# neobotix/neo_mpc_planner2

Measured on AMD Instinct MI355X. Metric: MPC solves/sec (control_steps=3, 500x500 costmap), higher is better.
Workload: dtype f64

## Files before the change

### neo_mpc_planner2_amd/csrc/neo_mpc_kernels.hip

```cpp
#include <hip/hip_runtime.h>
#include <hip/hip_ext.h>
#include <math.h>
#include <stdint.h>
#include <stdlib.h>

#include "neo_mpc_device.h"
#include "wave_ops.h"
#include "fast_math.h"
#include "solver_context.h"
#include "solver_rules.h"
#include "costmap.h"
#include "feasible_set.h"
#include "rollout.h"
#include "riccati.h"
#include "adjoint.h"
#include "tangent_cone.h"
#include "dense_newton.h"
#include "lbfgs.h"
#include "cell_scan.h"

namespace neo_mpc {
namespace {

constexpr int kStallIterations = NEO_RULE_STALL_ITERATIONS;
constexpr int kBlockedRun = NEO_RULE_BLOCKED_RUN;
constexpr double kBlockedStep = NEO_RULE_BLOCKED_STEP;
constexpr double kFinalFracGaussNewton = NEO_RULE_FINAL_FRAC_GN;
constexpr double kWindowStep = NEO_RULE_WINDOW_STEP;
constexpr int kClosingRun = NEO_RULE_CLOSING_RUN;
constexpr int kLateIteration = NEO_RULE_LATE_ITERATION;

#ifdef NEO_MPC_PHASE_TIMING
#ifdef NEO_MPC_SEGMENT_TIMING
#define NEO_SEGMENT_DECL unsigned long long seg_t0 = 0, seg_t1 = 0, seg_scan = 0, seg_scan_at = 0
#define NEO_SEGMENT(k) seg_t##k = wall_clock64()
#define NEO_SEGMENT_SCAN_BEGIN() seg_scan_at = wall_clock64(); seg_scan = seg_scan_at
#define NEO_SEGMENT_SCAN_END() seg_scan = wall_clock64() - seg_scan
#define NEO_SEGMENT_DUMP()                                                                                   \
  {                                                                                                          \
    SolveArgs ad;                                                                                            \
    fresh_args<kSteps, kStaticTile, kLayoutSteps, kRouted>(ad);                                              \
    const int nvd = 3 * ad.p.n;                                                                              \
    if (ad.solution && lane_again() == 0 && nvd >= 9) {                                                      \
      ad.solution[(size_t)b * nvd + 4] = (double)seg_t0; ad.solution[(size_t)b * nvd + 5] = (double)seg_t1;  \
      ad.solution[(size_t)b * nvd + 3] = (double)seg_scan; ad.solution[(size_t)b * nvd + 2] = (double)seg_scan_at; \
    }                                                                                                        \
  }
#else
#define NEO_SEGMENT_DECL
#define NEO_SEGMENT(k)
#define NEO_SEGMENT_SCAN_BEGIN()
#define NEO_SEGMENT_SCAN_END()
#define NEO_SEGMENT_DUMP()
#endif
#define NEO_WAVE_START const unsigned long long wave_t0 = wall_clock64()
#define NEO_WAVE_END_ARGS(args)                                                                     \
  if ((args).solution && lane == 0 && (args).p.n >= 3) {                                            \
    const int nvw = 3 * (args).p.n;                                                                \
    unsigned int hw_id, xcc_id;                                                                    \
    asm volatile("s_getreg_b32 %0, hwreg(HW_REG_HW_ID)" : "=s"(hw_id));                            \
    asm volatile("s_getreg_b32 %0, hwreg(HW_REG_XCC_ID)" : "=s"(xcc_id));                          \
    (args).solution[(size_t)b * nvw + 6] = (double)wave_t0;                                        \
    (args).solution[(size_t)b * nvw + 7] = (double)wall_clock64();                                 \
    (args).solution[(size_t)b * nvw + 8] = (double)hw_id + 4294967296.0 * (double)(xcc_id & 15u);  \
  }
#define NEO_PHASE_DECL long long phase_clock[8]
#define NEO_PHASE(k) phase_clock[k] = clock64()
#define NEO_PHASE_DUMP()                                                                            \
  if (it == 2 && a.solution && lane == 0)                                                          \
    for (int k = 0; k < 6; ++k) a.solution[(size_t)b * nv + k] = (double)(phase_clock[k + 1] - phase_clock[k])
#else
#define NEO_WAVE_START
#define NEO_WAVE_END_ARGS(args)
#define NEO_SEGMENT_DECL
#define NEO_SEGMENT(k)
#define NEO_SEGMENT_SCAN_BEGIN()
#define NEO_SEGMENT_SCAN_END()
#define NEO_SEGMENT_DUMP()
#define NEO_PHASE_DECL
#define NEO_PHASE(k)
#define NEO_PHASE_DUMP()
#endif
constexpr int kNewtonMaxSteps = 8;

constexpr int kRoutedSteps = 3;
constexpr LdsLayout make_routed_stagewise_layout() {
  LdsLayout l = make_lds_layout(kRoutedSteps, 0, true, true);
  constexpr LdsLayout dense = make_lds_layout(kRoutedSteps, 4, false);
  l.tile = dense.tile;
  l.total_bytes = dense.total_bytes;
  return l;
}
static_assert(make_lds_layout(kRoutedSteps, 0, true, true).tile <= make_lds_layout(kRoutedSteps, 4, false).tile,
              "the stage-wise arrays of three stages fit in front of the dense kernel's reach tile");
static_assert(make_lds_layout(kRoutedSteps, 0, true, true).gr == make_lds_layout(kRoutedSteps, 4, false).gr,
              "records, iterate and gradients share their offsets");
template <int kSteps, int kStaticTile, int kLayoutSteps, bool kRouted = false>
__device__ __forceinline__ void fresh_args(SolveArgs& a) {
  auto kp = (const __attribute__((address_space(4))) char*)__builtin_amdgcn_kernarg_segment_ptr();
  asm volatile("" : "+s"(kp));
  a = *(const SolveArgs*)kp;
  if (kRouted) {
    constexpr LdsLayout kLayout = make_routed_stagewise_layout();
    const int tile_w = a.lds.tile_w, tile_h = a.lds.tile_h, reach = a.lds.reach;
    a.lds = kLayout;
    a.lds.tile_w = tile_w; a.lds.tile_h = tile_h; a.lds.reach = reach;
    a.p.n = kRoutedSteps;
  } else if (kSteps || kStaticTile) {
    constexpr LdsLayout kStaticLayout = make_lds_layout(kLayoutSteps, kSteps ? 4 : 0, false);
    const int tile_w = a.lds.tile_w, tile_h = a.lds.tile_h, reach = a.lds.reach;
    a.lds = kStaticLayout;
    a.lds.tile_w = tile_w; a.lds.tile_h = tile_h; a.lds.reach = reach;
    if (kSteps) a.p.n = kSteps;
  }
}
__device__ __forceinline__ void own_loop_params(SolveArgs& a) {
  auto own = [](double& v) { asm volatile("" : "+s"(v)); };
  own(a.p.dt); own(a.p.wt_n); own(a.p.wo_n); own(a.p.wc_n); own(a.p.wterm_o); own(a.p.r);
  own(a.p.lo[2]); own(a.p.hi[2]);
  own(a.map.origin_x); own(a.map.origin_y); own(a.map.resolution); own(a.map.inv_resolution);
}
template <bool kVectorPose>
__device__ __forceinline__ void ctx_from_lds(const SolveArgs& a, const double* L, Ctx& c) {
  const double* P = L + a.lds.prob;
  const double* t = L + a.lds.tol;
  c.cx = lane_value(P[P_CARROT_X], 0); c.cy = lane_value(P[P_CARROT_Y], 0);
  c.tyaw = lane_value(t[T_TYAW], 0); c.fyaw = lane_value(t[T_FYAW], 0);
  c.v0 = lane_value(P[P_VEL], 0); c.v1 = lane_value(P[P_VEL + 1], 0); c.v2 = lane_value(P[P_VEL + 2], 0);
  c.c0 = t[T_C0]; c.s0 = t[T_S0]; c.X0 = P[P_CUR_X]; c.Y0 = P[P_CUR_Y];
  if (kVectorPose) asm volatile("" : "+v"(c.c0), "+v"(c.s0), "+v"(c.X0), "+v"(c.Y0));
  else { c.c0 = lane_value(c.c0, 0); c.s0 = lane_value(c.s0, 0); c.X0 = lane_value(c.X0, 0); c.Y0 = lane_value(c.Y0, 0); }
  const int* ti = reinterpret_cast<const int*>(t + T_TILE);
  c.tile_x0 = uniform_int(ti[0]); c.tile_y0 = uniform_int(ti[1]); c.tile_geom = uniform_int(ti[2]);
  c.konst = 0.0; c.true_yaw = 0.0;
}

struct SolveCarry {
  int flags;
  bool cold;
  bool wall_in_reach;
  double f = INFINITY;
  int it = 0, nfev = 1, status = NEO_MPC_STATUS_MAX_ITER;
};

template <int kSteps, bool kTame, int kStaticTile, int kLayoutSteps>
__device__ __forceinline__ bool solve_setup(double* L, uint32_t b, int lane, SolveCarry& s) {
  constexpr bool kCovered = kStaticTile > 0;
  int flags;
  bool cold = true;
  {
    SolveArgs a;
    fresh_args<kSteps, kStaticTile, kLayoutSteps>(a);
    const DevParams& p = a.p;
    const int n = kSteps ? kSteps : p.n, nv = 3 * n;
    load_records(a, L, b, lane);
    if (uniform_int(reinterpret_cast<const int*>(L + a.lds.prob)[PI_SKIP]) == 1) { skip_instance(a, b, lane); return false; }
    select_map(a.map, L + a.lds.prob);
    flags = reset_and_warm(a, L, b, lane) ? NEO_MPC_FLAG_RESET : 0;
    const double fcost = footprint_cost(a, L, b, lane);
    if (lane == 0) L[a.lds.prob + P_FOOTPRINT] = fcost;
    Ctx c;
    make_ctx_wave(p, a.map, L + a.lds.prob, fcost, c, lane);
    load_tile(a, c, L, lane);
    s.wall_in_reach = (c.tile_geom & kTileWall) != 0;
    if (s.wall_in_reach) flags |= NEO_MPC_FLAG_WALL_IN_REACH;
    if (lane == 0) {
      double* t = L + a.lds.tol;
      t[T_XTOL] = p.xtol; t[T_EARLY] = p.early_tol; t[T_FINAL] = p.final_tol; t[T_FTOL] = p.ftol;
      t[T_STALL] = p.stall_step; t[T_WTOL] = p.wtol; t[T_WTOL_LATE] = p.wtol_late; t[T_KINK] = p.kink_radius;
      t[T_KONST] = c.konst; t[T_TRUE_YAW] = c.true_yaw;
      t[T_HOP_DROP] = p.hop_min_drop; t[T_HOP_RANGE] = p.hop_range;
      t[T_BTOL_MAP] = p.btol_map; t[T_BTOL_FREE] = p.btol_free;
      reinterpret_cast<int*>(t + T_HOP_STAGE)[kHopLanes] = 0;
      t[T_C0] = c.c0; t[T_S0] = c.s0; t[T_TYAW] = c.tyaw; t[T_FYAW] = c.fyaw;
      int* ti = reinterpret_cast<int*>(t + T_TILE);
      ti[0] = c.tile_x0; ti[1] = c.tile_y0; ti[2] = c.tile_geom;
    }
    double* u = L + a.lds.u;
    for (int i = lane; i < n; i += kLanes) project_block<kTame>(p, u[3 * i], u[3 * i + 1], u[3 * i + 2]);
    WAVE_SYNC();
    for (int k = 0; k < nv; ++k) cold = cold && (u[k] == 0.0);
    ctx_from_lds<false>(a, L, c);
    {
      double* S = L + a.lds.state;
      int* Si = reinterpret_cast<int*>(S);
      const bool has_prev = uniform_int(Si[SI_HAS_PREV]) == 1 && !(flags & NEO_MPC_FLAG_RESET);
      WAVE_SYNC();
      if (lane == 0) {
        double q0 = has_prev ? S[S_PREV_U0] : u[nv - 3], q1 = has_prev ? S[S_PREV_U0 + 1] : u[nv - 2], q2 = has_prev ? S[S_PREV_U0 + 2] : u[nv - 1];
        project_block<kTame>(p, q0, q1, q2);
        S[S_PREV_U0] = q0; S[S_PREV_U0 + 1] = q1; S[S_PREV_U0 + 2] = q2;
        Si[SI_HAS_PREV] = 0;
      }
      WAVE_SYNC();
    }
    if (!cold && n > 1 && !(p.compat & kCompatNoUnshift) && p.max_it < kDumpGradient) {
      const double* A0 = L + a.lds.state + S_PREV_U0;
      double ts = 0.0;
      const double fs = rollout_cost<kSteps, kTame, kCovered>(
          a, c, L,
          [&](int i, double& b0, double& b1, double& b2) {
            const double* src = lane == 1 ? (i == 0 ? A0 : u + 3 * (i - 1)) : u + 3 * i;
            b0 = src[0]; b1 = src[1]; b2 = src[2];
          },
          NoRecord(), &ts);
      const double f_warm = lane_value(fs, 0), f_alt = lane_value(fs, 1);
      const bool free_both = lane_value(ts, 0) == 0.0 && lane_value(ts, 1) == 0.0;
      if (f_alt < f_warm && free_both) {
        double v0 = 0.0, v1 = 0.0, v2 = 0.0;
        const int k0 = lane, k1 = lane + kLanes, k2 = lane + 2 * kLanes;
        if (k0 < nv) v0 = k0 >= 3 ? u[k0 - 3] : A0[k0];
        if (k1 < nv) v1 = u[k1 - 3];
        if (k2 < nv) v2 = u[k2 - 3];
        WAVE_SYNC();
        if (k0 < nv) u[k0] = v0;
        if (k1 < nv) u[k1] = v1;
        if (k2 < nv) u[k2] = v2;
      } else if (f_alt < f_warm && lane == 0) {
        reinterpret_cast<int*>(L + a.lds.state)[SI_HAS_PREV] = kAltArmed;
      }
      WAVE_SYNC();
    }
  }
  s.flags = flags; s.cold = cold;
  return true;
}

template <int kMinWavesPerSimd, int kSteps, int kDir, bool kTame, int kStaticTile, int kLayoutSteps, bool kRouted = false>
__device__ __forceinline__ bool solve_search(double* L, uint32_t b, SolveCarry& sc) {
  constexpr bool kCovered = kStaticTile > 0;
  constexpr bool kNewton = kDir == 1;
  constexpr bool kRiccati = kDir == 2;
  constexpr bool kSecond = kDir != 0;
  constexpr bool kBlockedRule = kNewton || kRouted;
  static_assert(!kRiccati || kSteps == 0 || kRouted, "the stage-wise direction: run-time-sized, or the routed kernel's control_steps-3 branch");
  static_assert(!kRouted || (kRiccati && kSteps == kRoutedSteps), "the routed branch is the stage-wise one, three stages in registers");
  constexpr int kFew = (kRiccati && kSteps > 0) ? kSteps : 0;
  constexpr int kNwSteps = !kNewton ? 1 : kSteps ? kSteps : kNewtonMaxSteps;
  constexpr bool kVectorPose = kTame;
  constexpr int kRegSteps = kSteps ? kSteps : 1;
  constexpr int kPairs = kSteps ? 4 : NEO_MPC_MAX_LBFGS_MEMORY;
  double f = sc.f;
  const bool cold = sc.cold;
  int npairs = 0, head = 0, nfev = sc.nfev, it = sc.it, status = sc.status, stall = 0;
  int blocked_run = 0;
  int nblocked = 1;
  double u_term = 0.0;
  double gain1 = INFINITY, gain2 = INFINITY;
  bool final_step = false;
  double alpha = 1.0;
  bool scanned = false;
  int nscans = 0;
  bool scan_only = false;
  auto lane_again = []() {
    int zero;
    asm volatile("v_mov_b32 %0, 0" : "=v"(zero));
    return (int)__builtin_amdgcn_mbcnt_hi(~0u, __builtin_amdgcn_mbcnt_lo(~0u, (unsigned)zero));
  };
  NEO_SEGMENT_DECL;
  NEO_SEGMENT(0);
  for (;;) {
  SolveArgs a;
  fresh_args<kSteps, kStaticTile, kLayoutSteps, kRouted>(a);
  own_loop_params(a);
  select_map(a.map, L + a.lds.prob);
  const DevParams& p = a.p;
  const int n = kSteps ? kSteps : p.n, nv = 3 * n, mem = p.mem;
  double cand[3 * kRegSteps], cand_sn[kRegSteps], cand_cs[kRegSteps];
  bool have_trig = false;
  Ctx c;
  ctx_from_lds<kVectorPose>(a, L, c);
  double* u = L + a.lds.u;
  double* gs = L + a.lds.gs;
  double* gt = L + a.lds.gt;
  double* gr = L + a.lds.gr;
  double* d = L + a.lds.d;
  double* u_prev = L + a.lds.u_prev;
  double* gt_prev = L + a.lds.gt_prev;
  double* u_new = L + a.lds.u_new;
  double* ACS = L + a.lds.cs;
  double* ASN = L + a.lds.sn;
  int* AMODE = reinterpret_cast<int*>(L + a.lds.mode);
  static_assert(2 * 7 >= kNewtonRecord, "Newton records do not fit the step arrays");

  if (!scanned && nscans == 0) {
    const int lane = lane_again();
    for (int i = lane; i < n; i += kLanes) { AMODE[4 * i + 2] = 0; AMODE[4 * i + 3] = 0; }
    if (kRouted && lane == 0) L[a.lds.tol + T_KINK] = p.kink_radius_stagewise;
    alpha = kRiccati ? fmax(1.0, n * 0.125) : 1.0;
    if (kFew && lane == 0) { double* t = L + a.lds.tol; t[T_GAIN1] = INFINITY; t[T_GAIN2] = INFINITY; t[T_ALPHA] = alpha; }
    if (kRiccati && lane == 0) L[a.lds.tol + T_MU] = n > 8 ? (double)(n - 8) * 0.125 : 0.0;
  }
  bool v_feasible = false;
  if (kRiccati) {
    double b0 = c.v0, b1 = c.v1, b2 = c.v2;
    asm volatile("" : "+v"(b0), "+v"(b1), "+v"(b2));
    project_block<kTame>(p, b0, b1, b2);
    v_feasible = b0 == c.v0 && b1 == c.v1 && b2 == c.v2;
  }
  double my_scale;
  {
    int l0 = lane_again();
    my_scale = kRiccati ? 0.0 : lane_scale<kSecond>(l0);
  }
  for (; it < p.max_it && !scan_only; ++it) {
    int lane = lane_again();
    const bool exact_step = kRiccati && nblocked == 0;
    int tol_off = a.lds.tol;
    asm volatile("" : "+s"(tol_off));
    const double* TOL = L + tol_off;
    NEO_PHASE_DECL;
    NEO_PHASE(0);
    constexpr int kVars = 3 * kNwSteps;
    const int nvr = kSteps ? kVars : nv;
    bool free_path = false;
    int nhops = 0;
    float hc[kVars];
    float newton_sol = 0.0f;
    if (kNewton) {
      double hcol[kSteps ? kVars : 1];
      const double hstep = 1e-6, inv_h = 1.0 / hstep;
      double pcs[kNwSteps], psn[kNwSteps];
      double x = 0.0, y = 0.0, th = 0.0;
    #pragma unroll
      for (int i = 0; i < kNwSteps; ++i) {
        if (kSteps || i < n) {
          const double vx = u[3 * i] + (lane == 3 * i ? hstep : 0.0);
          const double vy = u[3 * i + 1] + (lane == 3 * i + 1 ? hstep : 0.0);
          const double w = u[3 * i + 2] + (lane == 3 * i + 2 ? hstep : 0.0);
          th += w * p.dt;
          sincos_heading<kTame>(th, &psn[i], &pcs[i]);
          x += (vx * pcs[i] - vy * psn[i]) * p.dt;
          y += (vx * psn[i] + vy * pcs[i]) * p.dt;
        }
      }
      double SX = 0.0, SY = 0.0, ST = 0.0;
    #pragma unroll
      for (int k = kNwSteps - 1; k >= 0; --k) {
        if (kSteps || k < n) {
          const double vx = u[3 * k] + (lane == 3 * k ? hstep : 0.0);
          const double vy = u[3 * k + 1] + (lane == 3 * k + 1 ? hstep : 0.0);
          const double w = u[3 * k + 2] + (lane == 3 * k + 2 ? hstep : 0.0);
          const double pdx = (vx * pcs[k] - vy * psn[k]) * p.dt, pdy = (vx * psn[k] + vy * pcs[k]) * p.dt;
          double prt = -2.0 * p.wo_n * (c.tyaw - th);
          if (k == n - 1) prt += -2.0 * p.wterm_o * (c.fyaw - th);
          SX += -2.0 * p.wt_n * (c.cx - x); SY += -2.0 * p.wt_n * (c.cy - y);
          ST += prt - pdy * SX + pdx * SY;
          const double g0 = p.dt * (pcs[k] * SX + psn[k] * SY), g1 = p.dt * (-psn[k] * SX + pcs[k] * SY),
                       g2 = p.dt * ST;
          if (kSteps) {
            hcol[3 * k] = g0; hcol[3 * k + 1] = g1; hcol[3 * k + 2] = g2;
          } else {
            const double b0 = lane_value(g0, 63), b1 = lane_value(g1, 63), b2 = lane_value(g2, 63);
            if (lane == 63) { gs[3 * k] = b0; gs[3 * k + 1] = b1; gs[3 * k + 2] = b2; }
            hc[3 * k] = (float)((g0 - b0) * inv_h);
            hc[3 * k + 1] = (float)((g1 - b1) * inv_h);
            hc[3 * k + 2] = (float)((g2 - b2) * inv_h);
          }
          x -= pdx; y -= pdy; th -= w * p.dt;
        } else {
          hc[3 * k] = 0.0f; hc[3 * k + 1] = 0.0f; hc[3 * k + 2] = 0.0f;
        }
      }
      if (kSteps) {
    #pragma unroll
        for (int j = 0; j < kVars; ++j) {
          const double base = lane_value(hcol[j], 63);
          if (lane == 63) gs[j] = base;
          hc[j] = (float)((hcol[j] - base) * inv_h);
        }
      }
      WAVE_SYNC();
    }
    else if (!kSteps || kRiccati) adjoint_by_scans<kTame, kRiccati, kFew>(a, c, L, exact_step, lane, n, free_path, nhops);
    else adjoint_short_sweep<kSteps, kTame>(a, c, L, have_trig, lane, n);
    NEO_PHASE(1);
    const bool my_corner = tangent_cone_pass<kTame, kNewton, kRiccati>(a, c, L, TOL[T_KINK], lane, n);
    WAVE_SYNC();
    const bool corner_any = kSecond && !kTame && __ballot(my_corner) != 0ull && (kRiccati ? free_path : (it > 0 && u_term == 0.0));
    NEO_PHASE(2);
    if (p.max_it == kDumpGradient) {
      for (int k = lane; k < nv; k += kLanes) a.solution[(size_t)b * nv + k] = gt[k];
      return true;
    }
    if (kSecond && it == 0 && cold) {
      if (kRiccati) { for (int k = lane; k < nv; k += kLanes) d[k] = -gr[k]; }
      else if (lane < nvr) d[lane] = -gr[lane];
      if (kRiccati) for (int i = lane; i < n; i += kLanes) AMODE[4 * i + 3] = 0;
      WAVE_SYNC();
    } else if (kRiccati) {
      riccati_prepare(a, c, L, n, lane, v_feasible, (float)TOL[T_MU]);
      WAVE_SYNC();
      if (corner_any) riccati_keep_linear_terms(a, L, n, lane, true);
      auto sweep = [&]() {
        riccati_sweep<float, (kMinWavesPerSimd < 4), kFew>(a, L, n, lane);
        riccati_finish(a, c, L, n, lane);
      };
      sweep();
      if (!kTame && corner_any && repin_corner_blocks<true>(a, L, n, lane)) {
        riccati_keep_linear_terms(a, L, n, lane, false);
        sweep();
      }
    } else if (kNewton) {
      newton_sol = dense_newton_direction<kSteps, kNwSteps, kTame>(a, L, hc, corner_any, lane, n, nvr);
    }
    NEO_PHASE(3);
    if (!kSecond) lbfgs_direction<kSteps, kPairs>(a, L, it, mem, head, npairs, lane, n);
    if (kSecond && it > 0) {
      float dm = 0.0f;
      int anynear = 0;
      if (kRiccati) {
        for (int k = lane; k < nv; k += kLanes) {
          const float v = (float)fabs(d[k]);
          dm = (v == v) ? fmaxf(dm, v) : INFINITY;
          anynear |= (AMODE[4 * (k / 3) + 2] == 1);
        }
      } else if (lane < nvr) { dm = fabsf(newton_sol); anynear = (AMODE[4 * (lane / 3) + 2] == 1); }
      dm = wave_max_f(dm);
      const bool near_any = __ballot(anynear != 0) != 0ull;
      if ((double)dm < TOL[T_EARLY] && !near_any && nhops == 0) { status = NEO_MPC_STATUS_CONVERGED; break; }
      if ((double)dm < ((kRiccati && !exact_step) ? kFinalFracGaussNewton : 1.0) * TOL[T_FINAL] && !near_any) final_step = true;
    }
    NEO_PHASE(4);
    if (p.max_it > kDumpGradient && it == p.max_it - kDumpGradient - 1) {
      for (int k = lane; k < nv; k += kLanes) a.solution[(size_t)b * nv + k] = d[k];
      return true;
    }
    const double lscale = kRiccati ? lane_scale<kSecond>(lane) : my_scale;
    const double alpha_now = kFew ? TOL[T_ALPHA] : alpha;
    const double pstep = alpha_now * lscale;
    const double step = lane < 32 ? pstep : lscale;
    constexpr double kTrialRatio = NEO_RULE_TRIAL_RATIO;
    bool took_trial = false;
    double fb = INFINITY, cterm = 0.0;
    int best = 32;
    if (kRiccati && free_path && it > 0) {
      const bool on = lane < n;
      double b0 = 0.0, b1 = 0.0, b2 = 0.0, g0 = 0.0, g1 = 0.0, g2 = 0.0;
      if (on) {
        candidate_block<kTame, kRiccati>(a, c, L, 32, 1.0, alpha_now, lane, b0, b1, b2);
        g0 = gr[3 * lane]; g1 = gr[3 * lane + 1]; g2 = gr[3 * lane + 2];
        u_new[3 * lane] = b0; u_new[3 * lane + 1] = b1; u_new[3 * lane + 2] = b2;
      }
      auto scan = [](double v) { if constexpr (kFew > 0) return wave_scan_few<kFew>(v); else return wave_scan(v); };
      auto sum = [](double v) { if constexpr (kFew > 0) return wave_sum_few<kFew>(v); else return wave_sum(v); };
      const double th = scan(b2 * p.dt);
      double sn, cs;
      sincos_heading<kTame>(th, &sn, &cs);
      const double x = scan((b0 * cs - b1 * sn) * p.dt), y = scan((b0 * sn + b1 * cs) * p.dt);
      double fi = 0.0, pr = 0.0, tm = 0.0;
      if (on) {
        const double dx = c.cx - x, dy = c.cy - y, et = c.tyaw - th;
        const double e0 = c.v0 - b0, e1 = c.v1 - b1, e2 = c.v2 - b2;
        tm = step_term<kCovered>(a, c, L, x, y);
        fi = p.wt_n * (dx * dx + dy * dy) + p.wo_n * (et * et) + p.wc_n * sqrt_fast(e0 * e0 + e1 * e1 + e2 * e2) + tm;
        if (lane == n - 1) { const double ef = c.fyaw - th; fi += p.wterm_o * (ef * ef); }
        pr = -0.5 * (g0 * (b0 - u[3 * lane]) + g1 * (b1 - u[3 * lane + 1]) + g2 * (b2 - u[3 * lane + 2]));
      }
      const double ft = sum(fi), pred = sum(pr);
      if (ft < f && f - ft >= kTrialRatio * pred) {
        took_trial = true; fb = ft;
        if (kBlockedRule) cterm = sum(tm);
      }
      WAVE_SYNC();
    }
    const double* ALT0 = L + a.lds.state + S_PREV_U0;
    bool alt_armed = false;
    if (it == 0) alt_armed = uniform_int(reinterpret_cast<const int*>(L + a.lds.state)[SI_HAS_PREV]) == kAltArmed;
    if (!took_trial) {
    int hop_stage = -1;
    float hop_x = 0.0f, hop_y = 0.0f;
    if (kRiccati && lane >= 1 && lane <= nhops) {
      const double* t = TOL;
      hop_stage = reinterpret_cast<const int*>(t + T_HOP_STAGE)[lane - 1];
      hop_x = reinterpret_cast<const float*>(t + T_HOP_VEC)[2 * (lane - 1)];
      hop_y = reinterpret_cast<const float*>(t + T_HOP_VEC)[2 * (lane - 1) + 1];
    }
    double fc = rollout_cost<kSteps, kTame, kCovered>(
        a, c, L,
        [&](int i, double& b0, double& b1, double& b2) {
          candidate_block<kTame, kRiccati>(a, c, L, lane, step, pstep, i, b0, b1, b2, hop_stage, hop_x, hop_y);
          if (it == 0) {
            asm volatile("");
            if (lane == 0) { b0 = u[3 * i]; b1 = u[3 * i + 1]; b2 = u[3 * i + 2]; }
            if (lane == kAltLane && alt_armed) { const double* src = i == 0 ? ALT0 : u + 3 * (i - 1); b0 = src[0]; b1 = src[1]; b2 = src[2]; }
          }
          if (kSteps) { cand[3 * i] = b0; cand[3 * i + 1] = b1; cand[3 * i + 2] = b2; }
        },
        [&](int i, double sn, double cs) {
          if (kSteps && !kSecond) { cand_sn[i] = sn; cand_cs[i] = cs; }
        }, kBlockedRule ? &cterm : nullptr);
    NEO_PHASE(5);
    if (!(fc == fc)) fc = INFINITY;
    if (it == 0) { f = lane_value(fc, 0); if (kNewton) u_term = lane_value(cterm, 0); }
    fb = fc;
    best = lane;
    wave_argmin(fb, best);
    }
    ++nfev;
    if (!(fb < f)) { status = NEO_MPC_STATUS_CONVERGED; ++it; break; }
    const bool alt_won = alt_armed && best == kAltLane;
    float stepmax = 0.0f;
    if (kSteps && kSecond && !took_trial) {
      if (lane == best) {
#pragma unroll
        for (int k = 0; k < 3 * kRegSteps; ++k) {
          stepmax = fmaxf(stepmax, (float)fabs(cand[k] - u[k]));
          u[k] = cand[k];
        }
      }
      stepmax = __builtin_bit_cast(float, __builtin_amdgcn_readlane(__builtin_bit_cast(int, stepmax), best));
      have_trig = true;
    } else {
      if (kSteps && !kSecond) {
        if (lane == best) {
#pragma unroll
          for (int i = 0; i < kRegSteps; ++i) {
            u_new[3 * i] = cand[3 * i]; u_new[3 * i + 1] = cand[3 * i + 1]; u_new[3 * i + 2] = cand[3 * i + 2];
            ASN[i] = cand_sn[i]; ACS[i] = cand_cs[i];
          }
        }
      } else if (!kSteps && !took_trial) {
        const double bstep = lane_value(step, best), bpstep = lane_value(pstep, best);
        int bhop = -1;
        float bhx = 0.0f, bhy = 0.0f;
        if (kRiccati && best >= 1 && best <= nhops) {
          bhop = reinterpret_cast<const int*>(TOL + T_HOP_STAGE)[best - 1];
          bhx = reinterpret_cast<const float*>(TOL + T_HOP_VEC)[2 * (best - 1)];
          bhy = reinterpret_cast<const float*>(TOL + T_HOP_VEC)[2 * (best - 1) + 1];
        }
        for (int i = lane; i < n; i += kLanes) {
          double b0, b1, b2;
          candidate_block<kTame, kRiccati>(a, c, L, best, bstep, bpstep, i, b0, b1, b2, bhop, bhx, bhy);
          if (alt_won) { const double* src = i == 0 ? ALT0 : u + 3 * (i - 1); b0 = src[0]; b1 = src[1]; b2 = src[2]; }
          u_new[3 * i] = b0; u_new[3 * i + 1] = b1; u_new[3 * i + 2] = b2;
        }
      }
      have_trig = true;
      WAVE_SYNC();
      for (int k = lane; k < nv; k += kLanes) {
        const double nu = u_new[k], ou = u[k];
        stepmax = fmaxf(stepmax, (float)fabs(nu - ou));
        if (!kSecond) { u_prev[k] = ou; gt_prev[k] = gt[k]; }
        u[k] = nu;
      }
      stepmax = wave_max_f(stepmax);
    }
    const double gain = f - fb;
    const double fscale = fmax(1.0, fabs(fb));
    stall = (gain <= TOL[T_FTOL] * fscale || (double)stepmax <= TOL[T_STALL]) ? stall + 1 : 0;
    const bool hop_won = (kRiccati && best >= 1 && best <= nhops) || alt_won;
    nblocked = (best < 32 || lane_value(step, best) < kWindowStep || hop_won) ? nblocked + 1 : 0;
    const bool window_on = !kRiccati || kRouted || nblocked >= 3;
    const double wtol0 = TOL[T_WTOL];
    const double wtol = it >= kLateIteration ? TOL[T_WTOL_LATE] : wtol0;
    const double g1 = kFew ? TOL[T_GAIN1] : gain1, g2 = kFew ? TOL[T_GAIN2] : gain2;
    bool creeping = wtol > 0.0 && gain + g1 + g2 <= wtol * fscale && window_on;
    bool free_now = kRiccati ? free_path : false;
    if (kNewton) free_now = lane_value(cterm, best) == 0.0;
    creeping = creeping || (wtol0 > 0.0 && (double)stepmax <= TOL[T_STALL] && gain <= 0.5 * g1 && g1 <= 0.5 * g2 &&
                            (!free_now || (g2 < INFINITY && gain * gain <= TOL[T_FTOL] * fscale * (g1 - gain))) &&
                            ((kRiccati && !kRouted) ? window_on : nblocked >= kClosingRun));
    bool blocked_stop = false;
    if (kBlockedRule) {
      const double bs = lane_value(step, best);
      blocked_run = (best < 32 || bs < kBlockedStep) ? blocked_run + 1 : 0;
      if (blocked_run >= kBlockedRun) {
        const bool free_rollout = lane_value(cterm, best) == 0.0;
        const double btol = free_rollout ? TOL[T_BTOL_FREE] : TOL[T_BTOL_MAP];
        blocked_stop = gain + g1 + g2 <= btol;
      }
    }
    double* TOLW = L + tol_off;
    if (kFew) { if (lane == 0) { TOLW[T_GAIN2] = g1; TOLW[T_GAIN1] = gain; } }
    else { gain2 = gain1; gain1 = gain; }
    f = fb;
    if (nblocked != 0) final_step = false;
    if (kNewton) u_term = lane_value(cterm, best);
    if (kRiccati && !(it == 0 && cold) && !hop_won) {
      constexpr unsigned long long kNearlyFull = newton_lanes_at_least(0.8), kShort = kNewtonLanes & ~newton_lanes_at_least(0.3);
      const double mu0 = n > 8 ? (double)(n - 8) * 0.125 : 0.0, mu = TOL[T_MU];
      double* mu_slot = L + tol_off + T_MU;
      if ((kNearlyFull >> best) & 1ull) { if (lane == 0) *mu_slot = fmax(0.25 * mu, mu0 * 0.0625); }
      else if (best < 32 || ((kShort >> best) & 1ull)) { if (lane == 0) *mu_slot = fmin(4.0 * mu, 16.0 * mu0); }
    }
    if (best < 32 && !hop_won) {
      const double al = clampd(lane_value(step, best), 1e-6, 1e6);
      if (kFew) { if (lane == 0) TOLW[T_ALPHA] = al; }
      else alpha = al;
    }
    WAVE_SYNC();
    NEO_PHASE(6);
    NEO_PHASE_DUMP();
    if ((double)stepmax < TOL[T_XTOL] || stall >= kStallIterations || creeping || final_step || blocked_stop) { status = NEO_MPC_STATUS_CONVERGED; ++it; break; }
  }

  if (!kSecond || scanned || status != NEO_MPC_STATUS_CONVERGED || p.max_it >= kDumpGradient) break;
  const bool nothing_to_scan = (c.tile_geom & kTileFree) || (kNewton && u_term == 0.0);
  if (nothing_to_scan && nscans == 0) break;
  bool resume = false;
  {
    SolveArgs as;
    fresh_args<kSteps, kStaticTile, kLayoutSteps, kRouted>(as);
    select_map(as.map, L + as.lds.prob);
    Ctx cs;
    ctx_from_lds<false>(as, L, cs);
    int ls = lane_again();
    if (nscans == 0 && ls == 0) L[as.lds.tol + T_FSCAN] = f;
    NEO_SEGMENT_SCAN_BEGIN();
    const bool w = !nothing_to_scan &&
                   cell_scan<kSteps, kTame, kCovered>(as, cs, L, f, kNewton ? &u_term : nullptr, nfev, ls, kSteps ? kSteps : as.p.n);
    NEO_SEGMENT_SCAN_END();
    ++nscans;
    scan_only = w && nscans < NEO_RULE_SCAN_REPEATS;
    if (!scan_only) {
      scanned = true;
      WAVE_SYNC();
      resume = L[as.lds.tol + T_FSCAN] - f > as.p.scan_resume_gain && it < as.p.max_it;
      if (kFew && resume) {
        if (ls == 0) { L[as.lds.tol + T_GAIN1] = INFINITY; L[as.lds.tol + T_GAIN2] = INFINITY; }
        WAVE_SYNC();
      }
    }
  }
  if (scan_only) continue;
  if (!resume) break;
  status = NEO_MPC_STATUS_MAX_ITER; stall = 0; final_step = false; blocked_run = 0; nblocked = 1;
  gain1 = INFINITY; gain2 = INFINITY;
  }
  NEO_SEGMENT(1);
  NEO_SEGMENT_DUMP();
  if (scanned && status == NEO_MPC_STATUS_MAX_ITER) status = NEO_MPC_STATUS_CONVERGED;
  sc.f = f; sc.it = it; sc.nfev = nfev; sc.status = status;
  return false;
}

template <int kSteps, int kStaticTile, int kLayoutSteps>
__device__ __forceinline__ void solve_finish(double* L, uint32_t b, int lane, const SolveCarry& sc) {
  const int flags = sc.flags, status = sc.status, it = sc.it, nfev = sc.nfev;
  double f = sc.f;
  SolveArgs a;
  fresh_args<kSteps, kStaticTile, kLayoutSteps>(a);
  select_map(a.map, L + a.lds.prob);
  const DevParams& p = a.p;
  const int n = kSteps ? kSteps : p.n, nv = 3 * n;
  double* u = L + a.lds.u;
  Ctx c;
  ctx_from_lds<false>(a, L, c);
#ifndef NEO_MPC_PHASE_TIMING
  if (a.solution && p.max_it < kDumpGradient)
    for (int k = lane; k < nv; k += kLanes) a.solution[(size_t)b * nv + k] = u[k];
#endif
  WAVE_SYNC();
  f += L[a.lds.tol + T_KONST];
  c.true_yaw = L[a.lds.tol + T_TRUE_YAW];
  postprocess(a, c, L, b, lane, u, status == NEO_MPC_STATUS_CONVERGED, L[a.lds.prob + P_FOOTPRINT], flags, f, status, it, nfev);
}

template <int kMinWavesPerSimd, int kSteps, int kDir = 0, bool kTame = false, int kStaticTile = 0>
__global__ __launch_bounds__(kLanes, kMinWavesPerSimd) void k_solve(const SolveArgs args) {
  extern __shared__ __align__(16) double Ldyn[];
  constexpr int kLayoutSteps = kSteps ? kSteps : kNewtonMaxSteps;
  constexpr LdsLayout kStaticLayout = make_lds_layout(kLayoutSteps, kSteps ? 4 : 0, false);
  constexpr int kStaticDoubles = kStaticTile ? (kStaticLayout.total_bytes + kStaticTile) / 8 : 2;
  __shared__ __align__(16) double Lstat[kStaticDoubles];
  double* const L = kStaticTile ? Lstat : Ldyn;
  const int lane = threadIdx.x;
  if (blockIdx.x >= args.count) return;
  const uint32_t b = args.order ? (uint32_t)__builtin_amdgcn_readfirstlane((int)args.order[blockIdx.x]) : blockIdx.x;
  if (b >= args.count) return;
  NEO_WAVE_START;
  SolveCarry sc;
  if (!solve_setup<kSteps, kTame, kStaticTile, kLayoutSteps>(L, b, lane, sc)) return;
  if (solve_search<kMinWavesPerSimd, kSteps, kDir, kTame, kStaticTile, kLayoutSteps>(L, b, sc)) return;
  solve_finish<kSteps, kStaticTile, kLayoutSteps>(L, b, lane, sc);
  NEO_WAVE_END_ARGS(args);
}

#ifdef NEO_MPC_TU_RICCATI
template <int kMinWavesPerSimd, bool kTame = false, int kStaticTile = 0>
__global__ __launch_bounds__(kLanes, kMinWavesPerSimd) void k_solve_routed(const SolveArgs args) {
  extern __shared__ __align__(16) double Ldyn[];
  constexpr int kSteps = kRoutedSteps;
  constexpr LdsLayout kStaticLayout = make_lds_layout(kSteps, 4, false);
  constexpr int kStaticDoubles = kStaticTile ? (kStaticLayout.total_bytes + kStaticTile) / 8 : 2;
  __shared__ __align__(16) double Lstat[kStaticDoubles];
  double* const L = kStaticTile ? Lstat : Ldyn;
  const int lane = threadIdx.x;
  if (blockIdx.x >= args.count) return;
  const uint32_t b = args.order ? (uint32_t)__builtin_amdgcn_readfirstlane((int)args.order[blockIdx.x]) : blockIdx.x;
  if (b >= args.count) return;
  NEO_WAVE_START;
  SolveCarry sc;
  if (!solve_setup<kSteps, kTame, kStaticTile, kSteps>(L, b, lane, sc)) return;
  if (__builtin_amdgcn_readfirstlane((int)sc.wall_in_reach)) {
    __builtin_amdgcn_s_setprio(3);
    if (solve_search<kMinWavesPerSimd, kSteps, 2, kTame, kStaticTile, kSteps, true>(L, b, sc)) return;
  } else {
    if (solve_search<kMinWavesPerSimd, kSteps, 1, kTame, kStaticTile, kSteps, false>(L, b, sc)) return;
  }
  solve_finish<kSteps, kStaticTile, kSteps>(L, b, lane, sc);
  NEO_WAVE_END_ARGS(args);
}
#endif

#ifndef NEO_MPC_TU_RICCATI
__global__ __launch_bounds__(kLanes) void k_postprocess(const SolveArgs args) {
  extern __shared__ __align__(16) double L[];
  SolveArgs a = args;
  const int lane = threadIdx.x;
  const uint32_t b = blockIdx.x;
  if (b >= a.count) return;
  const int nv = 3 * a.p.n;
  load_records(a, L, b, lane);
// ... 367 lines not shown
```

### neo_mpc_planner2_amd/csrc/riccati.h

```cpp
#pragma once
#include <hip/hip_runtime.h>
#include <math.h>
#include <stdint.h>

#include "neo_mpc_device.h"
#include "fast_math.h"
#include "solver_context.h"

namespace neo_mpc {
namespace {

enum : int {
  RS_PX = 0, RS_PY, RS_TX, RS_TY,
  RS_WXX, RS_WXY, RS_WYY, RS_FLAGS,
  RS_C00, RS_C01, RS_C02, RS_C11,
  RS_C12, RS_C22, RS_CS, RS_SN,
  RS_GT = 16,
  RS_GS = 19,
  RS_WK = 22,
  RS_WLX = 25, RS_WLY,
  RS_SY = 27,
  RS_GAIN = 16,
  kRicStage = 28
};
enum : int { RC_FREE3 = 0, RC_SLIDE_W, RC_XY, RC_SLIDE, RC_W, RC_NONE, RC_KINK, RF_CASE = 7, RF_KINK_OK = 8 };

typedef float ric_f4 __attribute__((ext_vector_type(4)));

__device__ __forceinline__ float ric_rcp(float x) { return __builtin_amdgcn_rcpf(x); }
__device__ __forceinline__ double ric_rcp(double x) { return rcp_fast(x); }
template <typename T> __device__ __forceinline__ T ric_max(T a, T b) { return a > b ? a : b; }
template <typename T> __device__ __forceinline__ T ric_abs(T a) { return a < (T)0 ? -a : a; }
__device__ __forceinline__ float ric_fma(float a, float b, float c) { return fmaf(a, b, c); }
__device__ __forceinline__ double ric_fma(double a, double b, double c) { return fma(a, b, c); }
template <typename T> __device__ __forceinline__ T ric_pivot(T p, T delta) { return p > delta ? p : ric_max(ric_abs(p), delta); }

__device__ __forceinline__ void riccati_prepare(const SolveArgs& a, const Ctx& c, double* L, int n, int lane,
                                                bool v_feasible, float mu) {
  if (lane >= n) return;
  const DevParams& p = a.p;
  float* rs = reinterpret_cast<float*>(L + a.lds.ric) + kRicStage * lane;
  const int* am = reinterpret_cast<const int*>(L + a.lds.mode) + 4 * lane;
  const double* gt = L + a.lds.gt + 3 * lane;
  const double* gs = L + a.lds.gs + 3 * lane;
  const double* u = L + a.lds.u + 3 * lane;
  const double cs = rs[RS_CS], sn = rs[RS_SN];
  const double idt = rcp_fast(p.dt);
  rs[RS_GT] = (float)((cs * gt[0] - sn * gt[1]) * idt); rs[RS_GT + 1] = (float)((sn * gt[0] + cs * gt[1]) * idt);
  rs[RS_GT + 2] = (float)(gt[2] * idt);
  rs[RS_GS] = (float)((cs * gs[0] - sn * gs[1]) * idt); rs[RS_GS + 1] = (float)((sn * gs[0] + cs * gs[1]) * idt);
  rs[RS_GS + 2] = (float)(gs[2] * idt);
  const double e0 = u[0] - c.v0, e1 = u[1] - c.v1, e2 = u[2] - c.v2;
  rs[RS_WK] = (float)(-(cs * e0 - sn * e1) * p.dt); rs[RS_WK + 1] = (float)(-(sn * e0 + cs * e1) * p.dt);
  rs[RS_WK + 2] = (float)(-e2 * p.dt);
  const double nx = L[a.lds.nx + lane], ny = L[a.lds.ny + lane];
  const double tx = -ny, ty = nx;
  const float rtx = (float)(cs * tx - sn * ty), rty = (float)(sn * tx + cs * ty);
  rs[RS_TX] = rtx; rs[RS_TY] = rty;
  const int near = am[2];
  const int xy = near ? 2 : am[0];
  const bool wfree = !(near || (am[1] & 1));
  const int kase = xy == 0 ? (wfree ? RC_FREE3 : RC_XY) : xy == 1 ? (wfree ? RC_SLIDE_W : RC_SLIDE) : (wfree ? RC_W : RC_NONE);
  const int flags = kase | ((!near && v_feasible) ? RF_KINK_OK : 0);
  rs[RS_FLAGS] = (float)flags;
  float c00 = 0.0f, c01 = 0.0f, c02 = 0.0f, c11 = 0.0f, c12 = 0.0f, c22 = 0.0f;
  if (!near) {
    const float f0 = (float)(cs * e0 - sn * e1), f1 = (float)(sn * e0 + cs * e1), f2 = (float)e2;
    const float fn2 = f0 * f0 + f1 * f1 + f2 * f2;
    const float ine = fn2 > 0.0f ? __builtin_amdgcn_rsqf(fn2) : 0.0f;
    const float i2 = (float)(idt * idt);
    const float sN = (float)p.wc_n * ine * i2, h0 = f0 * ine, h1 = f1 * ine, h2 = f2 * ine;
    const float k2 = reinterpret_cast<const float*>(L + a.lds.rt)[2 * lane] * i2;
    c00 = sN * (1.0f - h0 * h0) + k2 * rtx * rtx; c01 = -sN * h0 * h1 + k2 * rtx * rty; c02 = -sN * h0 * h2;
    c11 = sN * (1.0f - h1 * h1) + k2 * rty * rty; c12 = -sN * h1 * h2; c22 = sN * (1.0f - h2 * h2);
    const float mt = mu * (float)(2.0 * p.wt_n);
    c00 += mt; c11 += mt; c22 += mu * (float)(2.0 * p.wo_n);
  }
  rs[RS_C00] = c00; rs[RS_C01] = c01; rs[RS_C02] = c02; rs[RS_C11] = c11; rs[RS_C12] = c12; rs[RS_C22] = c22;
}

__device__ __forceinline__ void riccati_keep_linear_terms(const SolveArgs& a, double* L, int n, int lane, bool save) {
  ric_f4* rec = reinterpret_cast<ric_f4*>(reinterpret_cast<float*>(L + a.lds.ric) + kRicStage * lane + RS_GAIN);
  ric_f4* keep = reinterpret_cast<ric_f4*>(L + a.lds.keep) + 3 * lane;
  for (int i = lane; i < n; i += kLanes, rec += 7 * kLanes, keep += 3 * kLanes) {
    if (save) { keep[0] = rec[0]; keep[1] = rec[1]; keep[2] = rec[2]; }
    else { rec[0] = keep[0]; rec[1] = keep[1]; rec[2] = keep[2]; }
  }
  WAVE_SYNC();
}

template <typename T, bool kPrefetch = true, int kFew = 0>
__device__ __forceinline__ void riccati_sweep(const SolveArgs& a, double* L, int n, int lane) {
  const DevParams& p = a.p;
  float* RS = static_cast<float*>(__builtin_assume_aligned(reinterpret_cast<float*>(L + a.lds.ric), 16));
  int* AMODE = reinterpret_cast<int*>(L + a.lds.mode);
  double* d = L + a.lds.d;
  const float* ARTF = reinterpret_cast<const float*>(L + a.lds.rt);
  const T w2 = (T)(2.0 * p.wt_n), wo2 = (T)(2.0 * p.wo_n), wterm2 = (T)(2.0 * p.wterm_o);
  const T wc2 = (T)((p.wc_n * p.wc_n) / (p.dt * p.dt));

  T V00 = (T)0.0, V01 = (T)0.0, V02 = (T)0.0, V11 = (T)0.0, V12 = (T)0.0, V22 = (T)0.0, v0 = (T)0.0, v1 = (T)0.0, v2 = (T)0.0;
  ric_f4 r0, r1, r2, r3, r4, r5, r6;
  if (kPrefetch) {
    const ric_f4* R4 = reinterpret_cast<const ric_f4*>(RS + kRicStage * (n - 1));
    r0 = R4[0]; r1 = R4[1]; r2 = R4[2]; r3 = R4[3]; r4 = R4[4]; r5 = R4[5]; r6 = R4[6];
  }
  for (int i = (kFew ? kFew : n) - 1; i >= 0; --i) {
    const bool first = kFew > 0 && i == 0;
    if (!kPrefetch) {
      const ric_f4* R4 = reinterpret_cast<const ric_f4*>(RS + kRicStage * i);
      r0 = R4[0]; r1 = R4[1]; r2 = R4[2]; r3 = R4[3]; r4 = R4[4]; r5 = R4[5]; r6 = R4[6];
    }
    const T px = r0.x, py = r0.y, rtx = r0.z, rty = r0.w;
    const T wxx = r1.x, wxy = r1.y, wyy = r1.z;
    const int flags = __builtin_amdgcn_readfirstlane((int)r1.w);
    const T c00 = r2.x, c01 = r2.y, c02 = r2.z, c11 = r2.w, c12 = r3.x, c22 = r3.y;
    const T gt0 = r4.x, gt1 = r4.y, gt2 = r4.z, gs0 = r4.w, gs1 = r5.x, gs2 = r5.y, e0 = r5.z, e1 = r5.w, e2 = r6.x;
    v0 += (T)r6.y; v1 += (T)r6.z;
    const T sy = (T)r6.w, sx = (T)ARTF[2 * i + 1];
    if (kPrefetch && i > 0) {
      const ric_f4* R4 = reinterpret_cast<const ric_f4*>(RS + kRicStage * (i - 1));
      r0 = R4[0]; r1 = R4[1]; r2 = R4[2]; r3 = R4[3]; r4 = R4[4]; r5 = R4[5]; r6 = R4[6];
    }
    const T S00 = V00 + w2 + wxx, S01 = V01 + wxy, S11 = V11 + w2 + wyy;
    const T S22 = V22 + wo2 + (i == n - 1 ? wterm2 : (T)0.0);
    const T M02 = ric_fma(-py, S00, ric_fma(px, S01, V02));
    const T M12 = ric_fma(-py, S01, ric_fma(px, S11, V12));
    const T M22 = ric_fma(-py, M02, ric_fma(px, M12, ric_fma(-py, V02, ric_fma(px, V12, S22))));
    const T Z02 = M02 + sy, Z12 = M12 - sx, Z22 = M22 - ric_fma(sx, px, sy * py);
    const T z0 = v0, z1 = v1, z2 = ric_fma(-py, v0, ric_fma(px, v1, v2));
    T k0 = (T)0.0, k1 = (T)0.0, k2 = (T)0.0, K00 = (T)0.0, K01 = (T)0.0, K02 = (T)0.0, K10 = (T)0.0, K11 = (T)0.0, K12 = (T)0.0,
      K20 = (T)0.0, K21 = (T)0.0, K22 = (T)0.0;
    bool tokink = false;
    int kase = flags & RF_CASE;
    if (flags & RF_KINK_OK) {
      const T q0 = gs0 + z0 + S00 * e0 + S01 * e1 + Z02 * e2;
      const T q1 = gs1 + z1 + S01 * e0 + S11 * e1 + Z12 * e2;
      const T q2 = gs2 + z2 + Z02 * e0 + Z12 * e1 + Z22 * e2;
      if (__builtin_amdgcn_readfirstlane((int)(q0 * q0 + q1 * q1 + q2 * q2 <= wc2))) { tokink = true; kase = RC_KINK; }
    }
    const T q0 = gt0 + z0, q1 = gt1 + z1, q2 = gt2 + z2;
    switch (kase) {
      case RC_FREE3: {
        const T Q00 = S00 + c00, Q01 = S01 + c01, Q02 = Z02 + c02, Q11 = S11 + c11, Q12 = Z12 + c12, Q22 = Z22 + c22;
        const T delta = ric_max((T)1e-6 * ric_max(ric_abs(Q00), ric_max(ric_abs(Q11), ric_abs(Q22))), (T)1e-30);
        const T d0 = ric_pivot(Q00, delta), i0 = ric_rcp(d0);
        const T l10 = Q01 * i0, l20 = Q02 * i0;
        const T d1 = ric_pivot(Q11 - l10 * Q01, delta), i1 = ric_rcp(d1);
        const T h12 = Q12 - l20 * Q01;
        const T l21 = h12 * i1;
        const T d2 = ric_pivot(Q22 - l20 * Q02 - l21 * h12, delta), i2 = ric_rcp(d2);
#define NEO_RIC_SOLVE3(r0_, r1_, r2_, x0_, x1_, x2_)                                           \
        {                                                                                        \
          const T y0 = -(r0_), y1 = -(r1_) - l10 * y0, y2 = -(r2_) - l20 * y0 - l21 * y1;        \
          x2_ = y2 * i2;                                                                         \
          x1_ = y1 * i1 - l21 * x2_;                                                             \
          x0_ = y0 * i0 - l10 * x1_ - l20 * x2_;                                                 \
        }
        NEO_RIC_SOLVE3(q0, q1, q2, k0, k1, k2)
        if (first) break;
        NEO_RIC_SOLVE3(S00, S01, M02, K00, K10, K20)
        NEO_RIC_SOLVE3(S01, S11, M12, K01, K11, K21)
        NEO_RIC_SOLVE3(Z02, Z12, Z22, K02, K12, K22)
#undef NEO_RIC_SOLVE3
        v0 = z0 + S00 * k0 + S01 * k1 + M02 * k2;
        v1 = z1 + S01 * k0 + S11 * k1 + M12 * k2;
        v2 = z2 + Z02 * k0 + Z12 * k1 + Z22 * k2;
        V00 = S00 + S00 * K00 + S01 * K10 + M02 * K20;
        V01 = S01 + S00 * K01 + S01 * K11 + M02 * K21;
        V02 = M02 + S00 * K02 + S01 * K12 + M02 * K22;
        V11 = S11 + S01 * K01 + S11 * K11 + M12 * K21;
        V12 = M12 + S01 * K02 + S11 * K12 + M12 * K22;
        V22 = Z22 + Z02 * K02 + Z12 * K12 + Z22 * K22;
        break;
      }
      case RC_SLIDE_W:
      case RC_XY: {
        const bool bw = kase == RC_SLIDE_W;
        const T ax = bw ? rtx : (T)1.0, ay = bw ? rty : (T)0.0;
        const T Q00 = S00 + c00, Q01 = S01 + c01, Q11 = S11 + c11;
        const T Qa0 = ax * Q00 + ay * Q01, Qa1 = ax * Q01 + ay * Q11;
        const T haa = Qa0 * ax + Qa1 * ay;
        const T hab = bw ? ax * (Z02 + c02) + ay * (Z12 + c12) : Qa1;
        const T hbb = bw ? Z22 + c22 : Q11;
        const T ga = ax * q0 + ay * q1, gb = bw ? q2 : q1;
        const T Za0 = ax * S00 + ay * S01, Za1 = ax * S01 + ay * S11, Za2 = ax * Z02 + ay * Z12;
        const T Zb0 = bw ? M02 : S01, Zb1 = bw ? M12 : S11, Zb2 = bw ? Z22 : Z12;
        const T delta = ric_max((T)1e-6 * ric_max(ric_abs(haa), ric_abs(hbb)), (T)1e-30);
        const T d0 = ric_pivot(haa, delta), i0 = ric_rcp(d0);
        const T l = hab * i0;
        const T d1 = ric_pivot(hbb - l * hab, delta), i1 = ric_rcp(d1);
        T ka, kb, Ka0, Ka1, Ka2, Kb0, Kb1, Kb2;
#define NEO_RIC_SOLVE2(ra_, rb_, xa_, xb_)                       \
        {                                                          \
          const T y0 = -(ra_), y1 = -(rb_) - l * y0;               \
          xb_ = y1 * i1;                                           \
          xa_ = y0 * i0 - l * xb_;                                 \
        }
        NEO_RIC_SOLVE2(ga, gb, ka, kb)
        if (first) {
          k0 = ax * ka; k1 = ay * ka;
          if (bw) k2 = kb; else k1 = kb;
          break;
        }
        NEO_RIC_SOLVE2(Za0, Zb0, Ka0, Kb0)
        NEO_RIC_SOLVE2(Za1, Zb1, Ka1, Kb1)
        NEO_RIC_SOLVE2(Za2, Zb2, Ka2, Kb2)
#undef NEO_RIC_SOLVE2
        v0 = z0 + Za0 * ka + Zb0 * kb; v1 = z1 + Za1 * ka + Zb1 * kb; v2 = z2 + Za2 * ka + Zb2 * kb;
        V00 = S00 + Za0 * Ka0 + Zb0 * Kb0; V01 = S01 + Za0 * Ka1 + Zb0 * Kb1; V02 = M02 + Za0 * Ka2 + Zb0 * Kb2;
        V11 = S11 + Za1 * Ka1 + Zb1 * Kb1; V12 = M12 + Za1 * Ka2 + Zb1 * Kb2; V22 = Z22 + Za2 * Ka2 + Zb2 * Kb2;
        k0 = ax * ka; k1 = ay * ka; K00 = ax * Ka0; K01 = ax * Ka1; K02 = ax * Ka2; K10 = ay * Ka0; K11 = ay * Ka1; K12 = ay * Ka2;
        if (bw) { k2 = kb; K20 = Kb0; K21 = Kb1; K22 = Kb2; }
        else { k1 = kb; K10 = Kb0; K11 = Kb1; K12 = Kb2; }
        break;
      }
      case RC_SLIDE: {
        const T Q00 = S00 + c00, Q01 = S01 + c01, Q11 = S11 + c11;
        const T haa = (rtx * Q00 + rty * Q01) * rtx + (rtx * Q01 + rty * Q11) * rty;
        const T i0 = -ric_rcp(ric_pivot(haa, ric_max((T)1e-6 * ric_abs(haa), (T)1e-30)));
        const T Za0 = rtx * S00 + rty * S01, Za1 = rtx * S01 + rty * S11, Za2 = rtx * Z02 + rty * Z12;
        const T ka = (rtx * q0 + rty * q1) * i0, Ka0 = Za0 * i0, Ka1 = Za1 * i0, Ka2 = Za2 * i0;
        if (first) { k0 = rtx * ka; k1 = rty * ka; break; }
        v0 = z0 + Za0 * ka; v1 = z1 + Za1 * ka; v2 = z2 + Za2 * ka;
        V00 = S00 + Za0 * Ka0; V01 = S01 + Za0 * Ka1; V02 = M02 + Za0 * Ka2;
        V11 = S11 + Za1 * Ka1; V12 = M12 + Za1 * Ka2; V22 = Z22 + Za2 * Ka2;
        k0 = rtx * ka; k1 = rty * ka; K00 = rtx * Ka0; K01 = rtx * Ka1; K02 = rtx * Ka2; K10 = rty * Ka0; K11 = rty * Ka1; K12 = rty * Ka2;
        break;
      }
      case RC_W: {
        const T hbb = Z22 + c22;
        const T i0 = -ric_rcp(ric_pivot(hbb, ric_max((T)1e-6 * ric_abs(hbb), (T)1e-30)));
        k2 = q2 * i0;
        if (first) break;
        K20 = M02 * i0; K21 = M12 * i0; K22 = Z22 * i0;
        v0 = z0 + M02 * k2; v1 = z1 + M12 * k2; v2 = z2 + Z22 * k2;
        V00 = S00 + M02 * K20; V01 = S01 + M02 * K21; V02 = M02 + M02 * K22;
        V11 = S11 + M12 * K21; V12 = M12 + M12 * K22; V22 = Z22 + Z22 * K22;
        break;
      }
      case RC_KINK:
        k0 = e0; k1 = e1; k2 = e2;
        if (first) break;
        v0 = z0 + S00 * k0 + S01 * k1 + M02 * k2;
        v1 = z1 + S01 * k0 + S11 * k1 + M12 * k2;
        v2 = z2 + Z02 * k0 + Z12 * k1 + Z22 * k2;
        V00 = S00; V01 = S01; V02 = M02; V11 = S11; V12 = M12; V22 = Z22;
        break;
      default:
        v0 = z0; v1 = z1; v2 = z2;
        V00 = S00; V01 = S01; V02 = M02; V11 = S11; V12 = M12; V22 = Z22;
        break;
    }
    if (lane == 0) {
      ric_f4* G4 = reinterpret_cast<ric_f4*>(RS + kRicStage * i + RS_GAIN);
      G4[0] = ric_f4{(float)K00, (float)K01, (float)K02, (float)K10};
      G4[1] = ric_f4{(float)K11, (float)K12, (float)K20, (float)K21};
      G4[2] = ric_f4{(float)K22, (float)k0, (float)k1, (float)k2};
      AMODE[4 * i + 3] = tokink ? 1 : 0;
    }
  }
  WAVE_SYNC();
  T z0 = (T)0.0, z1 = (T)0.0, z2 = (T)0.0;
  for (int i = 0; i < n; ++i) {
    const ric_f4* R4 = reinterpret_cast<const ric_f4*>(RS + kRicStage * i);
    const ric_f4 s0 = R4[0], g0 = R4[4], g1 = R4[5], g2 = R4[6];
    const T w0 = (T)g2.y + (T)g0.x * z0 + (T)g0.y * z1 + (T)g0.z * z2;
    const T w1 = (T)g2.z + (T)g0.w * z0 + (T)g1.x * z1 + (T)g1.y * z2;
    const T w2f = (T)g2.w + (T)g1.z * z0 + (T)g1.w * z1 + (T)g2.x * z2;
    if (lane == 0) { d[3 * i] = (double)w0; d[3 * i + 1] = (double)w1; d[3 * i + 2] = (double)w2f; }
    const T e0 = z0 + w0, e1 = z1 + w1, e2 = z2 + w2f;
    z0 = ric_fma(-(T)s0.y, e2, e0); z1 = ric_fma((T)s0.x, e2, e1); z2 = e2;
  }
  WAVE_SYNC();
}

__device__ __forceinline__ void riccati_finish(const SolveArgs& a, const Ctx& c, double* L, int n, int lane) {
  if (lane < n) {
    const float* rs = reinterpret_cast<const float*>(L + a.lds.ric) + kRicStage * lane;
    const int* am = reinterpret_cast<const int*>(L + a.lds.mode) + 4 * lane;
    double* d = L + a.lds.d + 3 * lane;
    if (am[3]) {
      const double* u = L + a.lds.u + 3 * lane;
      d[0] = c.v0 - u[0]; d[1] = c.v1 - u[1]; d[2] = c.v2 - u[2];
    } else {
      const double cs = rs[RS_CS], sn = rs[RS_SN], idt = rcp_fast(a.p.dt);
      const double w0 = d[0], w1 = d[1], w2 = d[2];
      double d0 = (cs * w0 + sn * w1) * idt, d1 = (-sn * w0 + cs * w1) * idt;
      const int mode = am[2] ? 2 : am[0];
      if (mode == 1) {
        const double nx = L[a.lds.nx + lane], ny = L[a.lds.ny + lane];
        const double dot = d0 * nx + d1 * ny;
        d0 -= dot * nx; d1 -= dot * ny;
      } else if (mode == 2) { d0 = 0.0; d1 = 0.0; }
      d[0] = d0; d[1] = d1; d[2] = (am[2] || (am[1] & 1)) ? 0.0 : w2 * idt;
    }
  }
  WAVE_SYNC();
}

}
}
```

Measured before the change: 24.57 million.

## Keep few-stage Riccati forward-pass results in per-lane registers

For the fixed small-horizon case (kFew > 0), the backward sweep loop is fully unrolled. The forward pass loads every stage's gains into registers up front. Each lane then keeps its own stage's step in registers, and a new finish routine uses that value directly instead of re-reading d from LDS after lane 0 wrote it. The convergence check reads the per-lane direction from registers, so one LDS round trip and its wave sync are avoided. In exchange, register pressure rises and the few-stage and general paths now diverge in code.

```diff
diff --git a/neo_mpc_planner2_amd/csrc/neo_mpc_kernels.hip b/neo_mpc_planner2_amd/csrc/neo_mpc_kernels.hip
--- a/neo_mpc_planner2_amd/csrc/neo_mpc_kernels.hip
+++ b/neo_mpc_planner2_amd/csrc/neo_mpc_kernels.hip
@@ -317,6 +317,8 @@
     int nhops = 0;
     float hc[kVars];
     float newton_sol = 0.0f;
+    double dir0 = 0.0, dir1 = 0.0, dir2 = 0.0;
+    int dir_near = 0;
     if (kNewton) {
       double hcol[kSteps ? kVars : 1];
       const double hstep = 1e-6, inv_h = 1.0 / hstep;
@@ -393,8 +395,14 @@
       WAVE_SYNC();
       if (corner_any) riccati_keep_linear_terms(a, L, n, lane, true);
       auto sweep = [&]() {
-        riccati_sweep<float, (kMinWavesPerSimd < 4), kFew>(a, L, n, lane);
-        riccati_finish(a, c, L, n, lane);
+        if constexpr (kFew > 0) {
+          RicLaneStep mine = {};
+          riccati_sweep<float, (kMinWavesPerSimd < 4), kFew>(a, L, n, lane, &mine);
+          riccati_finish_few(a, c, L, n, lane, mine, dir0, dir1, dir2, dir_near);
+        } else {
+          riccati_sweep<float, (kMinWavesPerSimd < 4), kFew>(a, L, n, lane);
+          riccati_finish(a, c, L, n, lane);
+        }
       };
       sweep();
       if (!kTame && corner_any && repin_corner_blocks<true>(a, L, n, lane)) {
@@ -409,7 +417,15 @@
     if (kSecond && it > 0) {
       float dm = 0.0f;
       int anynear = 0;
-      if (kRiccati) {
+      if (kFew > 0) {
+        if (lane < n) {
+          for (const double dk : {dir0, dir1, dir2}) {
+            const float v = (float)fabs(dk);
+            dm = (v == v) ? fmaxf(dm, v) : INFINITY;
+          }
+          anynear = dir_near == 1;
+        }
+      } else if (kRiccati) {
         for (int k = lane; k < nv; k += kLanes) {
           const float v = (float)fabs(d[k]);
           dm = (v == v) ? fmaxf(dm, v) : INFINITY;
diff --git a/neo_mpc_planner2_amd/csrc/riccati.h b/neo_mpc_planner2_amd/csrc/riccati.h
--- a/neo_mpc_planner2_amd/csrc/riccati.h
+++ b/neo_mpc_planner2_amd/csrc/riccati.h
@@ -26,6 +26,8 @@
 enum : int { RC_FREE3 = 0, RC_SLIDE_W, RC_XY, RC_SLIDE, RC_W, RC_NONE, RC_KINK, RF_CASE = 7, RF_KINK_OK = 8 };
 
 typedef float ric_f4 __attribute__((ext_vector_type(4)));
+
+struct RicLaneStep { float w0, w1, w2; };
 
 __device__ __forceinline__ float ric_rcp(float x) { return __builtin_amdgcn_rcpf(x); }
 __device__ __forceinline__ double ric_rcp(double x) { return rcp_fast(x); }
@@ -90,7 +92,8 @@
 }
 
 template <typename T, bool kPrefetch = true, int kFew = 0>
-__device__ __forceinline__ void riccati_sweep(const SolveArgs& a, double* L, int n, int lane) {
+__device__ __forceinline__ void riccati_sweep(const SolveArgs& a, double* L, int n, int lane, RicLaneStep* mine = nullptr) {
+  static_assert(kFew <= 4, "the forward sweep holds every stage's gains in registers at once");
   const DevParams& p = a.p;
   float* RS = static_cast<float*>(__builtin_assume_aligned(reinterpret_cast<float*>(L + a.lds.ric), 16));
   int* AMODE = reinterpret_cast<int*>(L + a.lds.mode);
@@ -105,6 +108,7 @@
     const ric_f4* R4 = reinterpret_cast<const ric_f4*>(RS + kRicStage * (n - 1));
     r0 = R4[0]; r1 = R4[1]; r2 = R4[2]; r3 = R4[3]; r4 = R4[4]; r5 = R4[5]; r6 = R4[6];
   }
+#pragma unroll
   for (int i = (kFew ? kFew : n) - 1; i >= 0; --i) {
     const bool first = kFew > 0 && i == 0;
     if (!kPrefetch) {
@@ -262,6 +266,24 @@
   }
   WAVE_SYNC();
   T z0 = (T)0.0, z1 = (T)0.0, z2 = (T)0.0;
+  if constexpr (kFew > 0) {
+    ric_f4 s0[kFew], g0[kFew], g1[kFew], g2[kFew];
+#pragma unroll
+    for (int i = 0; i < kFew; ++i) {
+      const ric_f4* R4 = reinterpret_cast<const ric_f4*>(RS + kRicStage * i);
+      s0[i] = R4[0]; g0[i] = R4[4]; g1[i] = R4[5]; g2[i] = R4[6];
+    }
+#pragma unroll
+    for (int i = 0; i < kFew; ++i) {
+      const T w0 = (T)g2[i].y + (T)g0[i].x * z0 + (T)g0[i].y * z1 + (T)g0[i].z * z2;
+      const T w1 = (T)g2[i].z + (T)g0[i].w * z0 + (T)g1[i].x * z1 + (T)g1[i].y * z2;
+      const T w2f = (T)g2[i].w + (T)g1[i].z * z0 + (T)g1[i].w * z1 + (T)g2[i].x * z2;
+      if (lane == i) { mine->w0 = (float)w0; mine->w1 = (float)w1; mine->w2 = (float)w2f; }
+      const T e0 = z0 + w0, e1 = z1 + w1, e2 = z2 + w2f;
+      z0 = ric_fma(-(T)s0[i].y, e2, e0); z1 = ric_fma((T)s0[i].x, e2, e1); z2 = e2;
+    }
+    return;
+  }
   for (int i = 0; i < n; ++i) {
     const ric_f4* R4 = reinterpret_cast<const ric_f4*>(RS + kRicStage * i);
     const ric_f4 s0 = R4[0], g0 = R4[4], g1 = R4[5], g2 = R4[6];
@@ -299,5 +321,34 @@
   WAVE_SYNC();
 }
 
-}
-}
+__device__ __forceinline__ void riccati_finish_few(const SolveArgs& a, const Ctx& c, double* L, int n, int lane,
+                                                   const RicLaneStep& mine, double& o0, double& o1, double& o2, int& near) {
+  o0 = 0.0; o1 = 0.0; o2 = 0.0; near = 0;
+  if (lane < n) {
+    const float* rs = reinterpret_cast<const float*>(L + a.lds.ric) + kRicStage * lane;
+    const int* am = reinterpret_cast<const int*>(L + a.lds.mode) + 4 * lane;
+    double* d = L + a.lds.d + 3 * lane;
+    const int m0 = am[0], m1 = am[1], m2 = am[2];
+    near = m2;
+    if (am[3]) {
+      const double* u = L + a.lds.u + 3 * lane;
+      o0 = c.v0 - u[0]; o1 = c.v1 - u[1]; o2 = c.v2 - u[2];
+    } else {
+      const double cs = rs[RS_CS], sn = rs[RS_SN], idt = rcp_fast(a.p.dt);
+      const double w0 = (double)mine.w0, w1 = (double)mine.w1, w2 = (double)mine.w2;
+      double d0 = (cs * w0 + sn * w1) * idt, d1 = (-sn * w0 + cs * w1) * idt;
+      const int mode = m2 ? 2 : m0;
+      if (mode == 1) {
+        const double nx = L[a.lds.nx + lane], ny = L[a.lds.ny + lane];
+        const double dot = d0 * nx + d1 * ny;
+        d0 -= dot * nx; d1 -= dot * ny;
+      } else if (mode == 2) { d0 = 0.0; d1 = 0.0; }
+      o0 = d0; o1 = d1; o2 = (m2 || (m1 & 1)) ? 0.0 : w2 * idt;
+    }
+    d[0] = o0; d[1] = o1; d[2] = o2;
+  }
+  WAVE_SYNC();
+}
+
+}
+}
```

New measurement: 24.87 million (median of 6 runs). No clear change (+1.2%).
